# LFY1998/IPDM-PyTorch

Measured on AMD Instinct MI355X. Metric: CT slices/s (full proj+img partial-diffusion sample), higher is better.
Workload: dtype f32

## Files before the change

### ipdm-pytorch_amd/csrc/attn_bx3.hip

```cpp
#include "unet_kernels.h"
#include "attn_common.h"

using namespace ipdm;
using namespace ipdm::attn;

typedef float f32x16 __attribute__((ext_vector_type(16)));
typedef unsigned u32x4 __attribute__((ext_vector_type(4)));
typedef __bf16 bf16x8 __attribute__((ext_vector_type(8)));
typedef __bf16 bf16x2 __attribute__((ext_vector_type(2)));

namespace {

constexpr int D = 64;
constexpr int KT = 32;
constexpr int KP = 72;
constexpr int VP = 40;
constexpr int KPLANE = KT * KP, VPLANE = D * VP;
constexpr int STAGE = 3 * KPLANE + 3 * VPLANE;
constexpr int PCHUNK = 256;
constexpr int TILE_CHUNKS = 6 * PCHUNK;

__device__ inline unsigned pk_bf16(float a, float b)
{
    return __builtin_bit_cast(unsigned, bf16x2{(__bf16)a, (__bf16)b});
}
struct Split3 { unsigned h[3]; };
__device__ inline Split3 split3(float a, float b)
{
    Split3 s;
    s.h[0] = pk_bf16(a, b);
    const float ra = a - __builtin_bit_cast(float, s.h[0] << 16), rb = b - __builtin_bit_cast(float, s.h[0] & 0xffff0000u);
    s.h[1] = pk_bf16(ra, rb);
    const float qa = ra - __builtin_bit_cast(float, s.h[1] << 16), qb = rb - __builtin_bit_cast(float, s.h[1] & 0xffff0000u);
    s.h[2] = pk_bf16(qa, qb);
    return s;
}

__device__ inline f32x16 mma(u32x4 a, u32x4 b, f32x16 c)
{
    return __builtin_amdgcn_mfma_f32_32x32x16_bf16(__builtin_bit_cast(bf16x8, a), __builtin_bit_cast(bf16x8, b), c, 0, 0, 0);
}
template <bool FIRST>
__device__ inline f32x16 mma6(const u32x4 (&a)[3], const u32x4 (&b)[3], f32x16 c)
{
    if (FIRST) {
        const f32x16 zero = {0, 0, 0, 0, 0, 0, 0, 0, 0, 0, 0, 0, 0, 0, 0, 0};
        c = mma(a[0], b[2], zero);
        asm volatile("" ::"v"(a[0]), "v"(b[2]));
    } else {
        c = mma(a[0], b[2], c);
    }
    c = mma(a[2], b[0], c);
    c = mma(a[1], b[1], c);
    c = mma(a[0], b[1], c);
    c = mma(a[1], b[0], c);
    return mma(a[0], b[0], c);
}

__global__ void __launch_bounds__(256) attention_presplit_kernel(const float *__restrict__ qkv, u32x4 *__restrict__ planes, int heads, int T)
{
    constexpr int FP = KT + 1;
    __shared__ float kf[D * FP], vf[D * FP];
    const int bh = blockIdx.y, b = bh / heads, head = bh % heads;
    const float *qp = qkv + ((size_t)b * heads * 3 * D + (size_t)head * 3 * D) * T;
    const int s0 = blockIdx.x * KT, tid = threadIdx.x;
    {
        const int key = tid & 31, c0 = tid >> 5;
        const bool in = s0 + key < T;
#pragma unroll
        for (int r = 0; r < 8; ++r) {
            const int c = c0 + 8 * r;
            kf[c * FP + key] = in ? qp[(size_t)(D + c) * T + s0 + key] : 0.0f;
            vf[c * FP + key] = in ? qp[(size_t)(2 * D + c) * T + s0 + key] : 0.0f;
        }
    }
    __syncthreads();
    u32x4 *pt = planes + ((size_t)bh * gridDim.x + blockIdx.x) * TILE_CHUNKS + tid;
    const int ks = tid >> 3, kg = tid & 7, vc = tid >> 2, vg = tid & 3;
    const int vkey = 16 * (vg >> 1) + 4 * (vg & 1);
    u32x4 hk[3], hv[3];
#pragma unroll
    for (int e = 0; e < 8; e += 2) {
        const Split3 sk = split3(kf[(8 * kg + e) * FP + ks], kf[(8 * kg + e + 1) * FP + ks]);
        const Split3 sv = split3(vf[vc * FP + vkey + 8 * (e >> 2) + (e & 3)], vf[vc * FP + vkey + 8 * (e >> 2) + (e & 3) + 1]);
#pragma unroll
        for (int p = 0; p < 3; ++p) { hk[p][e / 2] = sk.h[p]; hv[p][e / 2] = sv.h[p]; }
    }
#pragma unroll
    for (int p = 0; p < 3; ++p) {
        pt[p * PCHUNK] = hk[p];
        pt[(3 + p) * PCHUNK] = hv[p];
    }
}

template <bool ZSEQ, bool PRE>
__global__ void __launch_bounds__(384, 3) attention_bx3_kernel(const float *__restrict__ qkv, float *__restrict__ out, int heads, int T,
                                                                float scale, int zsplit, float *__restrict__ part, int zseq,
                                                                const u32x4 *__restrict__ planes)
{
    __shared__ __attribute__((aligned(16))) unsigned short lds[2 * STAGE];
    const int bh = blockIdx.y;
    const int b = bh / heads, head = bh % heads;
    const float *qp = qkv + ((size_t)b * heads * 3 * D + (size_t)head * 3 * D) * T;
    const int ntiles = (T + KT - 1) / KT;
    const int nslice = ZSEQ ? zseq : zsplit;
    const int tps = 2 * (((T + 63) / 64 + nslice - 1) / nslice);
    const int it0 = ZSEQ ? 0 : blockIdx.z * tps, it1 = ZSEQ ? ntiles : min(ntiles, it0 + tps);

    if (__builtin_amdgcn_readfirstlane(threadIdx.x >> 6) >= 4) {
        if constexpr (PRE) {
            const int tid = threadIdx.x - 256;
            const __amdgpu_buffer_rsrc_t rs = __builtin_amdgcn_make_buffer_rsrc((void *)(planes + (size_t)bh * ntiles * TILE_CHUNKS), 0,
                                                                                  ntiles * TILE_CHUNKS * 16, 0x00020000);
            int ko[2], vo[2];
#pragma unroll
            for (int n = 0; n < 2; ++n) {
                const int j = tid + 128 * n;
                ko[n] = (j >> 3) * KP + 8 * (j & 7);
                vo[n] = 3 * KPLANE + (j >> 2) * VP + 8 * (j & 3);
            }
            u32x4 r[12];
            const auto load = [&](int it) {
#pragma unroll
                for (int i = 0; i < 12; ++i)
                    r[i] = __builtin_bit_cast(u32x4, __builtin_amdgcn_raw_buffer_load_b128(rs, tid * 16, (it * TILE_CHUNKS + 128 * i) * 16, 0));
            };
            const auto store = [&](int it) {
                unsigned short *st = lds + (it & 1) * STAGE;
#pragma unroll
                for (int i = 0; i < 6; ++i) {
                    *reinterpret_cast<u32x4 *>(st + (i >> 1) * KPLANE + ko[i & 1]) = r[i];
                    *reinterpret_cast<u32x4 *>(st + (i >> 1) * VPLANE + vo[i & 1]) = r[6 + i];
                }
            };
            if (it0 < it1) load(it0);
            for (int it = it0; it < it1; ++it) {
                store(it);
                if (it + 1 < it1) load(it + 1);
                __syncthreads();
            }
            return;
        }
        const int tid = threadIdx.x - 256;
        const __amdgpu_buffer_rsrc_t rs = __builtin_amdgcn_make_buffer_rsrc((void *)qp, 0, 3 * D * T * 4, 0x00020000);
        int ks[2], kg[2], koff[2], vg[2], vc[2], vkey[2], voff[2];
#pragma unroll
        for (int n = 0; n < 2; ++n) {
            const int idx = tid + 128 * n;
            ks[n] = idx & 31;
            kg[n] = idx >> 5;
            koff[n] = (8 * kg[n] * T + ks[n]) * 4;
            vg[n] = idx & 3;
            vc[n] = idx >> 2;
            vkey[n] = 16 * (vg[n] >> 1) + 4 * (vg[n] & 1);
            voff[n] = (vc[n] * T + vkey[n]) * 4;
        }
        float kr[2][8], vr[2][8];
        const auto load = [&](int it) {
            const int s0 = it * KT;
            if (s0 + KT <= T) {
#pragma unroll
                for (int n = 0; n < 2; ++n)
#pragma unroll
                    for (int e = 0; e < 8; ++e) {
                        kr[n][e] = __builtin_bit_cast(float, __builtin_amdgcn_raw_buffer_load_b32(rs, koff[n], (D * T + s0 + e * T) * 4, 0));
                        vr[n][e] = __builtin_bit_cast(float, __builtin_amdgcn_raw_buffer_load_b32(rs, voff[n], (2 * D * T + s0 + 8 * (e >> 2) + (e & 3)) * 4, 0));
                    }
            } else {
#pragma unroll
                for (int n = 0; n < 2; ++n)
#pragma unroll
                    for (int e = 0; e < 8; ++e) {
                        const int ko = s0 + ks[n] >= T ? 0x7fffffff : koff[n];
                        const int vo = s0 + vkey[n] + 8 * (e >> 2) + (e & 3) >= T ? 0x7fffffff : voff[n];
                        kr[n][e] = __builtin_bit_cast(float, __builtin_amdgcn_raw_buffer_load_b32(rs, ko, (D * T + s0 + e * T) * 4, 0));
                        vr[n][e] = __builtin_bit_cast(float, __builtin_amdgcn_raw_buffer_load_b32(rs, vo, (2 * D * T + s0 + 8 * (e >> 2) + (e & 3)) * 4, 0));
                    }
            }
        };
        const auto store = [&](int it) {
            unsigned short *st = lds + (it & 1) * STAGE;
#pragma unroll
            for (int n = 0; n < 2; ++n) {
                u32x4 hk[3], hv[3];
#pragma unroll
                for (int e = 0; e < 8; e += 2) {
                    const Split3 sk = split3(kr[n][e], kr[n][e + 1]), sv = split3(vr[n][e], vr[n][e + 1]);
#pragma unroll
                    for (int p = 0; p < 3; ++p) { hk[p][e / 2] = sk.h[p]; hv[p][e / 2] = sv.h[p]; }
                }
#pragma unroll
                for (int p = 0; p < 3; ++p) {
                    *reinterpret_cast<u32x4 *>(st + p * KPLANE + ks[n] * KP + 8 * kg[n]) = hk[p];
                    *reinterpret_cast<u32x4 *>(st + 3 * KPLANE + p * VPLANE + vc[n] * VP + 8 * vg[n]) = hv[p];
                }
            }
        };
        if (it0 < it1) load(it0);
        for (int it = it0; it < it1; ++it) {
            store(it);
            if (it + 1 < it1) load(it + 1);
            __syncthreads();
        }
        return;
    }

    const int tid = threadIdx.x, lane = tid & 63, wave = tid >> 6;
    const int l31 = lane & 31, lh = lane >> 5;
    const int t = blockIdx.x * 128 + wave * 32 + l31;
    u32x4 q[4][3];
#pragma unroll
    for (int kb = 0; kb < 4; ++kb) {
        float x[8];
#pragma unroll
        for (int e = 0; e < 8; ++e) x[e] = t < T ? qp[(size_t)(16 * kb + 8 * lh + e) * T + t] * (scale * scale) : 0.0f;
#pragma unroll
        for (int e = 0; e < 8; e += 2) {
            const Split3 s = split3(x[e], x[e + 1]);
#pragma unroll
            for (int p = 0; p < 3; ++p) q[kb][p][e / 2] = s.h[p];
        }
    }
    f32x16 o[2];
#pragma unroll
    for (int cb = 0; cb < 2; ++cb)
#pragma unroll
        for (int r = 0; r < 16; ++r) o[cb][r] = 0.0f;
    float m_run = -INFINITY, l_run = 0.0f;
    f32x16 num[ZSEQ ? 2 : 1];
    float M_all = -INFINITY, den = 0.0f;
#pragma unroll
    for (int cb = 0; cb < (ZSEQ ? 2 : 1); ++cb)
#pragma unroll
        for (int r = 0; r < 16; ++r) num[cb][r] = 0.0f;
    int slice_end = it0 + tps;
    u32x4 v[2][3] = {}, pp[2][3] = {};
    const auto reserve = [&]() {
        asm volatile("" ::"v"(v[0][0]), "v"(v[0][1]), "v"(v[0][2]), "v"(v[1][0]), "v"(v[1][1]), "v"(v[1][2]), "v"(pp[1][0]), "v"(pp[1][1]), "v"(pp[1][2]));
    };

    for (int it = it0; it < it1; ++it) {
        const int s0 = it * KT;
        __syncthreads();
        reserve();
        const unsigned short *st = lds + (it & 1) * STAGE;
        f32x16 sacc;
        u32x4 k[3];
        {
            const unsigned short *krow = st + l31 * KP + 8 * lh;
#pragma unroll
            for (int kb = 0; kb < 4; ++kb) {
#pragma unroll
                for (int p = 0; p < 3; ++p) k[p] = *reinterpret_cast<const u32x4 *>(krow + p * KPLANE + 16 * kb);
                sacc = kb == 0 ? mma6<true>(k, q[kb], sacc) : mma6<false>(k, q[kb], sacc);
            }
        }
        __builtin_amdgcn_sched_barrier(0);
        if (s0 + KT > T) {
#pragma unroll
            for (int r = 0; r < 16; ++r)
                if (s0 + crow(r, lh) >= T) sacc[r] = -INFINITY;
        }
        float mx = sacc[0];
#pragma unroll
        for (int r = 1; r < 16; ++r) mx = fmaxf(mx, sacc[r]);
        mx = halves_max(mx);
        const float m_new = fmaxf(m_run, mx);
        const float alpha = __builtin_amdgcn_exp2f((m_run - m_new) * LOG2E);
        float rs0 = 0.0f, rs1 = 0.0f;
#pragma unroll
        for (int r = 0; r < 16; r += 2) {
            sacc[r] = __builtin_amdgcn_exp2f((sacc[r] - m_new) * LOG2E);
            sacc[r + 1] = __builtin_amdgcn_exp2f((sacc[r + 1] - m_new) * LOG2E);
            rs0 += sacc[r];
            rs1 += sacc[r + 1];
        }
        const float rs = halves_sum(rs0 + rs1);
        asm volatile("" ::"v"(k[0]), "v"(k[1]), "v"(k[2]));
        l_run = l_run * alpha + rs;
        m_run = m_new;
        if (__any(alpha != 1.0f)) {
#pragma unroll
            for (int cb = 0; cb < 2; ++cb)
#pragma unroll
                for (int r = 0; r < 16; ++r) o[cb][r] *= alpha;
        }
#pragma unroll
        for (int kb = 0; kb < 2; ++kb)
#pragma unroll
            for (int e = 0; e < 8; e += 2) {
                const Split3 s = split3(sacc[8 * kb + e], sacc[8 * kb + e + 1]);
#pragma unroll
                for (int p = 0; p < 3; ++p) pp[kb][p][e / 2] = s.h[p];
            }
        __builtin_amdgcn_sched_barrier(0);
#pragma unroll
        for (int cb = 0; cb < 2; ++cb) {
            const unsigned short *vrow = st + 3 * KPLANE + (cb * 32 + l31) * VP + 8 * lh;
#pragma unroll
            for (int kb = 0; kb < 2; ++kb)
#pragma unroll
                for (int p = 0; p < 3; ++p) v[kb][p] = *reinterpret_cast<const u32x4 *>(vrow + p * VPLANE + 16 * kb);
#pragma unroll
            for (int kb = 0; kb < 2; ++kb) o[cb] = mma6<false>(v[kb], pp[kb], o[cb]);
        }
        __builtin_amdgcn_sched_barrier(0);
        if constexpr (ZSEQ) if (it + 1 == slice_end || it + 1 == it1) {
            const SliceWeights w = slice_weights(M_all, m_run);
            den = slice_fold(den, l_run, w);
#pragma unroll
            for (int cb = 0; cb < 2; ++cb)
#pragma unroll
                for (int r = 0; r < 16; ++r) { num[cb][r] = slice_fold(num[cb][r], o[cb][r], w); o[cb][r] = 0.0f; }
            m_run = -INFINITY;
            l_run = 0.0f;
            slice_end += tps;
        }
    }
    if (t >= T) { reserve(); return; }
    if (zsplit > 1) {
        float *pq = part + ((size_t)blockIdx.z * gridDim.y + bh) * (D + 2) * T;
#pragma unroll
        for (int cb = 0; cb < 2; ++cb)
#pragma unroll
            for (int r = 0; r < 16; ++r) pq[(size_t)(cb * 32 + crow(r, lh)) * T + t] = o[cb][r];
        if (lh == 0) { pq[(size_t)D * T + t] = m_run; pq[(size_t)(D + 1) * T + t] = l_run; }
        reserve();
        return;
    }
    float *op = out + ((size_t)b * heads * D + (size_t)head * D) * T;
    const float inv = 1.0f / (ZSEQ ? den : l_run);
#pragma unroll
    for (int cb = 0; cb < 2; ++cb)
#pragma unroll
        for (int r = 0; r < 16; ++r) op[(size_t)(cb * 32 + crow(r, lh)) * T + t] = (ZSEQ ? num[ZSEQ ? cb : 0][r] : o[cb][r]) * inv;
    reserve();
}

}

namespace ipdm {

size_t attention_planes_floats(int B, int heads, int d, int T)
{
    if (d != D || opt(OPT_ATTN_EXACT_F32) || opt(OPT_ATTN_LEGACY) || opt(OPT_ATTN_NO_PRESPLIT)) return 0;
    return (size_t)B * heads * cdiv(T, KT) * TILE_CHUNKS * 4;
}

void attention_bx3_launch(const float *qkv, float *out, int B, int heads, int T, float scale, int Z, bool seq, float *scratch,
                          float *planes, hipStream_t st)
{
    const dim3 grid(cdiv(T, 128), B * heads, seq ? 1 : Z);
    u32x4 *pl = reinterpret_cast<u32x4 *>(planes);
    if (pl) hipLaunchKernelGGL(attention_presplit_kernel, dim3(cdiv(T, KT), B * heads), dim3(256), 0, st, qkv, pl, heads, T);
    if (seq) {
        if (pl) hipLaunchKernelGGL((attention_bx3_kernel<true, true>), grid, dim3(384), 0, st, qkv, out, heads, T, scale, 1, (float *)nullptr, Z, pl);
        else hipLaunchKernelGGL((attention_bx3_kernel<true, false>), grid, dim3(384), 0, st, qkv, out, heads, T, scale, 1, (float *)nullptr, Z, pl);
    } else {
        if (pl) hipLaunchKernelGGL((attention_bx3_kernel<false, true>), grid, dim3(384), 0, st, qkv, out, heads, T, scale, Z, scratch, 1, pl);
        else hipLaunchKernelGGL((attention_bx3_kernel<false, false>), grid, dim3(384), 0, st, qkv, out, heads, T, scale, Z, scratch, 1, pl);
    }
}

}
```

### ipdm-pytorch_amd/csrc/common.h

```cpp
#pragma once
#include <hip/hip_runtime.h>
#include <cstdarg>
#include <cstdio>
#include <cstring>
#include <string>
#include <vector>
#include "../../include/ipdm_hip.h"

namespace ipdm {

void set_error(const char *fmt, ...);

#define IPDM_HIP_CHECK(expr)                                                                   \
    do {                                                                                       \
        hipError_t e_ = (expr);                                                                \
        if (e_ != hipSuccess) {                                                                \
            ipdm::set_error("%s failed: %s (%s:%d)", #expr, hipGetErrorString(e_), __FILE__,  \
                            __LINE__);                                                         \
            return IPDM_ERR_HIP;                                                               \
        }                                                                                      \
    } while (0)

#define IPDM_REQUIRE(cond, ...)                   \
    do {                                          \
        if (!(cond)) {                            \
            ipdm::set_error(__VA_ARGS__);         \
            return IPDM_ERR_INVALID;              \
        }                                         \
    } while (0)

#define IPDM_LAUNCH_CHECK() IPDM_HIP_CHECK(hipGetLastError())

static inline int cdiv(long a, long b) { return (int)((a + b - 1) / b); }
static inline size_t align_up(size_t v, size_t a) { return (v + a - 1) / a * a; }

enum Opt {
    OPT_CONV_NO_UP2,
    OPT_CONV_NO_WUP2,
    OPT_CONV_LEGACY, OPT_CONV1X1_LEGACY, OPT_CONVS2_LEGACY,
    OPT_CONV_NO_DIRECT, OPT_DIRECT_NO_PLANAR, OPT_DIRECT_MAX_CIN, OPT_DIRECT_NO_S2, OPT_DIRECT_NO_SKIP_FUSE,
    OPT_CONV_DBG, OPT_CONV_VEC4_STRICT, OPT_CONV_NO_SPLITK, OPT_CONV_NO_WINO, OPT_WINO_V1, OPT_WINO2_MIN_TILES, OPT_CONV1X1_NO_QUARTER, OPT_CONV_NO_PW, OPT_PW_ITEM, OPT_PW_FORCE,
    OPT_CONV_NM,
    OPT_GN_TWO_STAGE, OPT_GN_UNFUSED,
    OPT_UNET_TRANSPOSE,
    OPT_ATTN_NO_KVSPLIT, OPT_ATTN_LEGACY, OPT_ATTN_NO_ZSEQ,
    OPT_ART_PER_VIEW,
    OPT_CONV_BF16X3,
    OPT_ATTN_EXACT_F32,
    OPT_ATTN_NO_PRESPLIT,
    OPT_COUNT
};
int opt(Opt o);
bool opt_per_call(int o);
const char *opt_name(int o);
void opt_snapshot(int (&dst)[OPT_COUNT]);
int opt_changed_since(const int (&rec)[OPT_COUNT]);
std::vector<int> opt_per_call_values();

int ensure_dynamic_lds(const void *kernel, size_t bytes);
int device_cu_count();

int unet_io_channels(const ipdm_unet *net, int *cin, int *cout);

__device__ inline double wave_sum(double v)
{
#pragma unroll
    for (int o = 32; o > 0; o >>= 1) v += __shfl_down(v, o, 64);
    return v;
}
__device__ inline float wave_sum(float v)
{
#pragma unroll
    for (int o = 32; o > 0; o >>= 1) v += __shfl_down(v, o, 64);
    return v;
}
__device__ inline float wave_max(float v)
{
#pragma unroll
    for (int o = 32; o > 0; o >>= 1) v = fmaxf(v, __shfl_down(v, o, 64));
    return v;
}

}
```

### ipdm-pytorch_amd/csrc/common.hip

```cpp
#include <cctype>
#include <cstdlib>
#include <mutex>
#include <strings.h>
#include <set>
#include <utility>
#include "common.h"

namespace ipdm {
static thread_local char g_err[512] = "";
void set_error(const char *fmt, ...)
{
    va_list ap;
    va_start(ap, fmt);
    vsnprintf(g_err, sizeof(g_err), fmt, ap);
    va_end(ap);
}

namespace {
std::mutex g_attr_mu;
std::set<std::pair<const void *, int>> g_attr_done;
int g_cus[64];
}

namespace {
struct OptDef { const char *name; int def; bool per_call; int lo = 0, hi = 1; };
const OptDef g_opt_def[OPT_COUNT] = {
    {"conv_no_up2", 0, true},
    {"conv_no_wup2", 0, true},
    {"conv_legacy", 0, false}, {"conv1x1_legacy", 0, false}, {"convs2_legacy", 0, false},
    {"conv_no_direct", 0, false}, {"direct_no_planar", 0, false},
    {"direct_max_cin", 160, false, 0, 160},
    {"direct_no_s2", 0, false}, {"direct_no_skip_fuse", 0, true},
    {"conv_dbg", 0, true, 0, 0x3ff}, {"conv_vec4_strict", 0, false}, {"conv_no_splitk", 0, false},
    {"conv_no_wino", 0, true}, {"wino_v1", 0, true}, {"wino2_min_tiles", 192, true, 0, 1 << 24},
    {"conv1x1_no_quarter", 0, true}, {"conv_no_pw", 0, true}, {"pw_item", 0, true, 0, 2}, {"pw_force", 0, true}, {"conv_nm", 0, true, 0, 2},
    {"gn_two_stage", 0, true}, {"gn_unfused", 0, true},
    {"unet_transpose", -1, true, -1, 1},
    {"attn_no_kvsplit", 0, false}, {"attn_legacy", 0, false}, {"attn_no_zseq", 0, true},
    {"art_per_view", 0, true},
    {"conv_bf16x3", 0, true},
    {"attn_exact_f32", 0, true},
    {"attn_no_presplit", 0, true},
};
bool opt_value_ok(int i, int v)
{
    return v >= g_opt_def[i].lo && v <= g_opt_def[i].hi;
}
std::mutex g_opt_mu;
int g_opt_val[OPT_COUNT];
bool g_opt_init = false;

void opt_init_locked()
{
    if (g_opt_init) return;
    for (int i = 0; i < OPT_COUNT; ++i) {
        char env[64] = "IPDM_";
        size_t n = 5;
        for (const char *c = g_opt_def[i].name; *c && n + 1 < sizeof(env); ++c) env[n++] = (char)toupper((unsigned char)*c);
        env[n] = 0;
        const char *e = getenv(env);
        g_opt_val[i] = g_opt_def[i].def;
        if (e) {
            char *end = nullptr;
            const long v = strtol(e, &end, 10);
            const int want = (end != e) ? (int)v : 1;
            if (opt_value_ok(i, want)) g_opt_val[i] = want;
            else fprintf(stderr, "libipdm_hip: %s=%s is outside the option's range [%d, %d]: ignored\n", env, e, g_opt_def[i].lo, g_opt_def[i].hi);
        }
    }
    g_opt_init = true;
}
}

int opt(Opt o)
{
    std::lock_guard<std::mutex> lk(g_opt_mu);
    opt_init_locked();
    return g_opt_val[o];
}
bool opt_per_call(int o) { return g_opt_def[o].per_call; }
const char *opt_name(int o) { return g_opt_def[o].name; }
void opt_snapshot(int (&dst)[OPT_COUNT])
{
    std::lock_guard<std::mutex> lk(g_opt_mu);
    opt_init_locked();
    for (int i = 0; i < OPT_COUNT; ++i) dst[i] = g_opt_val[i];
}
std::vector<int> opt_per_call_values()
{
    std::lock_guard<std::mutex> lk(g_opt_mu);
    opt_init_locked();
    std::vector<int> v;
    for (int i = 0; i < OPT_COUNT; ++i)
        if (g_opt_def[i].per_call) v.push_back(g_opt_val[i]);
    return v;
}
int opt_changed_since(const int (&rec)[OPT_COUNT])
{
    std::lock_guard<std::mutex> lk(g_opt_mu);
    opt_init_locked();
    for (int i = 0; i < OPT_COUNT; ++i)
        if (!g_opt_def[i].per_call && g_opt_val[i] != rec[i]) return i;
    return -1;
}
static int opt_find(const char *name)
{
    if (!name) return -1;
    if (!strncmp(name, "IPDM_", 5) || !strncmp(name, "ipdm_", 5)) name += 5;
    for (int i = 0; i < OPT_COUNT; ++i)
        if (!strcasecmp(name, g_opt_def[i].name)) return i;
    return -1;
}

int ensure_dynamic_lds(const void *kernel, size_t bytes)
{
    int dev = 0;
    IPDM_HIP_CHECK(hipGetDevice(&dev));
    std::lock_guard<std::mutex> lk(g_attr_mu);
    if (g_attr_done.count({kernel, dev})) return IPDM_OK;
    IPDM_HIP_CHECK(hipFuncSetAttribute(kernel, hipFuncAttributeMaxDynamicSharedMemorySize, (int)bytes));
    g_attr_done.insert({kernel, dev});
    return IPDM_OK;
}

int device_cu_count()
{
    int dev = 0, v = 0;
    if (hipGetDevice(&dev) != hipSuccess || dev < 0 || dev >= 64) return 256;
    std::lock_guard<std::mutex> lk(g_attr_mu);
    if (!g_cus[dev])
        g_cus[dev] = (hipDeviceGetAttribute(&v, hipDeviceAttributeMultiprocessorCount, dev) == hipSuccess && v > 0) ? v : 256;
    return g_cus[dev];
}
}

extern "C" const char *ipdm_last_error(void) { return ipdm::g_err; }
extern "C" int ipdm_abi_version(void) { return IPDM_ABI_VERSION; }

extern "C" int ipdm_set_option(const char *name, int value)
{
    const int i = ipdm::opt_find(name);
    IPDM_REQUIRE(i >= 0, "ipdm_set_option: unknown option '%s'", name ? name : "(null)");
    IPDM_REQUIRE(ipdm::opt_value_ok(i, value), "ipdm_set_option: %s = %d is outside [%d, %d]", ipdm::g_opt_def[i].name, value,
                 ipdm::g_opt_def[i].lo, ipdm::g_opt_def[i].hi);
    std::lock_guard<std::mutex> lk(ipdm::g_opt_mu);
    ipdm::opt_init_locked();
    ipdm::g_opt_val[i] = value;
    return IPDM_OK;
}

extern "C" int ipdm_get_option(const char *name, int *value)
{
    const int i = ipdm::opt_find(name);
    IPDM_REQUIRE(i >= 0 && value, "ipdm_get_option: unknown option '%s'", name ? name : "(null)");
    *value = ipdm::opt((ipdm::Opt)i);
    return IPDM_OK;
}
```

Before: 2.161.

## Software-pipeline attention loop: overlap next tile's QK^T with current softmax and PV

Adds a pipelined variant of the bf16x3 attention kernel for the presplit, non-sequential path. The producer warps now stage K and V halves of each tile one barrier apart. The compute warps interleave the next tile's QK^T MMAs with the current tile's exp/split and PV MMAs, using sched_barrier pinning and register-reservation asm. The goal is to hide softmax and LDS latency behind matrix work. The cost is more register pressure and complex scheduling, and an env option can disable it.

After: 2.187 (median of 6 runs). 1.2% higher.

```diff
diff --git a/ipdm-pytorch_amd/csrc/attn_bx3.hip b/ipdm-pytorch_amd/csrc/attn_bx3.hip
--- a/ipdm-pytorch_amd/csrc/attn_bx3.hip
+++ b/ipdm-pytorch_amd/csrc/attn_bx3.hip
@@ -1,5 +1,7 @@
 #include "unet_kernels.h"
 #include "attn_common.h"
+#include "attn_pipe_schedule.h"
+#include <type_traits>
 
 using namespace ipdm;
 using namespace ipdm::attn;
@@ -57,6 +59,15 @@
     return mma(a[0], b[0], c);
 }
 
+template <int FROM, int TO, class F>
+__device__ inline void static_for(F &&f)
+{
+    if constexpr (FROM < TO) {
+        f(std::integral_constant<int, FROM>{});
+        static_for<FROM + 1, TO>(f);
+    }
+}
+
 __global__ void __launch_bounds__(256) attention_presplit_kernel(const float *__restrict__ qkv, u32x4 *__restrict__ planes, int heads, int T)
 {
     constexpr int FP = KT + 1;
@@ -93,11 +104,13 @@
     }
 }
 
-template <bool ZSEQ, bool PRE>
+template <bool ZSEQ, bool PRE, bool PIPE>
 __global__ void __launch_bounds__(384, 3) attention_bx3_kernel(const float *__restrict__ qkv, float *__restrict__ out, int heads, int T,
                                                                 float scale, int zsplit, float *__restrict__ part, int zseq,
                                                                 const u32x4 *__restrict__ planes)
 {
+    static_assert(PRE || !PIPE, "the pipelined loop copies planes");
+    static_assert(!ZSEQ || !PIPE, "the pipelined loop does not fit the slice walk's registers");
     __shared__ __attribute__((aligned(16))) unsigned short lds[2 * STAGE];
     const int bh = blockIdx.y;
     const int b = bh / heads, head = bh % heads;
@@ -106,6 +119,7 @@
     const int nslice = ZSEQ ? zseq : zsplit;
     const int tps = 2 * (((T + 63) / 64 + nslice - 1) / nslice);
     const int it0 = ZSEQ ? 0 : blockIdx.z * tps, it1 = ZSEQ ? ntiles : min(ntiles, it0 + tps);
+    const int npipe = max(it1 - it0, 0);
 
     if (__builtin_amdgcn_readfirstlane(threadIdx.x >> 6) >= 4) {
         if constexpr (PRE) {
@@ -133,6 +147,34 @@
                     *reinterpret_cast<u32x4 *>(st + (i >> 1) * VPLANE + vo[i & 1]) = r[6 + i];
                 }
             };
+            if constexpr (PIPE) {
+                const auto load_half = [&](int it, int h) {
+#pragma unroll
+                    for (int i = 6 * h; i < 6 * h + 6; ++i)
+                        r[i] = __builtin_bit_cast(u32x4, __builtin_amdgcn_raw_buffer_load_b128(rs, tid * 16, (it * TILE_CHUNKS + 128 * i) * 16, 0));
+                };
+                const auto store_k = [&](int it) {
+                    unsigned short *st = lds + attn_pipe::slot(it) * STAGE;
+#pragma unroll
+                    for (int i = 0; i < 6; ++i) *reinterpret_cast<u32x4 *>(st + (i >> 1) * KPLANE + ko[i & 1]) = r[i];
+                };
+                const auto store_v = [&](int it) {
+                    unsigned short *st = lds + attn_pipe::slot(it) * STAGE;
+#pragma unroll
+                    for (int i = 0; i < 6; ++i) *reinterpret_cast<u32x4 *>(st + (i >> 1) * VPLANE + vo[i & 1]) = r[6 + i];
+                };
+                if (npipe > 0) load_half(attn_pipe::k_stored(it0, npipe, 0), 0);
+                for (int b = 0; b < attn_pipe::barriers(npipe); ++b) {
+                    const int ks = attn_pipe::k_stored(it0, npipe, b), vs = attn_pipe::v_stored(it0, npipe, b);
+                    if (ks != attn_pipe::NONE) store_k(ks);
+                    if (vs != attn_pipe::NONE) store_v(vs);
+                    const int kl = attn_pipe::k_loaded(it0, npipe, b), vl = attn_pipe::v_loaded(it0, npipe, b);
+                    if (kl != attn_pipe::NONE) load_half(kl, 0);
+                    if (vl != attn_pipe::NONE) load_half(vl, 1);
+                    __syncthreads();
+                }
+                return;
+            }
             if (it0 < it1) load(it0);
             for (int it = it0; it < it1; ++it) {
                 store(it);
@@ -239,6 +281,135 @@
         asm volatile("" ::"v"(v[0][0]), "v"(v[0][1]), "v"(v[0][2]), "v"(v[1][0]), "v"(v[1][1]), "v"(v[1][2]), "v"(pp[1][0]), "v"(pp[1][1]), "v"(pp[1][2]));
     };
 
+    if constexpr (PIPE) {
+        f32x16 sacc = {};
+        float mx_c = 0.0f, m_new_c = 0.0f, alpha_c = 1.0f;
+        const auto row_max_alpha = [&]() {
+            mx_c = sacc[0];
+#pragma unroll
+            for (int r = 1; r < 16; ++r) mx_c = fmaxf(mx_c, sacc[r]);
+            mx_c = halves_max(mx_c);
+            m_new_c = fmaxf(m_run, mx_c);
+            alpha_c = __builtin_amdgcn_exp2f((m_run - m_new_c) * LOG2E);
+        };
+        u32x4 ka[2] = {}, pb[2] = {};
+        const auto interval = [&](auto has_s, auto has_pv, int b) {
+            constexpr bool HAS_S = decltype(has_s)::value, HAS_PV = decltype(has_pv)::value;
+            constexpr bool PIN = HAS_PV;
+            const int it = attn_pipe::v_read(it0, npipe, b), s0 = it * KT;
+            f32x16 snext;
+            u32x4 k[3], k0n;
+            if constexpr (HAS_PV) asm volatile("" ::"v"(ka[0]), "v"(ka[1]), "v"(pb[0]), "v"(pb[1]));
+            const unsigned short *krow = lds + (HAS_S ? attn_pipe::slot(attn_pipe::k_read(it0, npipe, b)) : 0) * STAGE + l31 * KP + 8 * lh;
+            const auto kterm = [&](int p, int kb) { return *reinterpret_cast<const u32x4 *>(krow + p * KPLANE + 16 * kb); };
+            float rs0 = 0.0f, rs1 = 0.0f;
+            float ra[4], rb[4];
+            unsigned h0[4];
+            const auto split_a = [&](int kb, int i) {
+                const float x = sacc[8 * kb + 2 * i], y = sacc[8 * kb + 2 * i + 1];
+                h0[i] = pk_bf16(x, y);
+                ra[i] = x - __builtin_bit_cast(float, h0[i] << 16);
+                rb[i] = y - __builtin_bit_cast(float, h0[i] & 0xffff0000u);
+            };
+            const auto split_b = [&](int kb, int i) {
+                const unsigned h1 = pk_bf16(ra[i], rb[i]);
+                const float qa = ra[i] - __builtin_bit_cast(float, h1 << 16), qb = rb[i] - __builtin_bit_cast(float, h1 & 0xffff0000u);
+                pp[kb][0][i] = h0[i];
+                pp[kb][1][i] = h1;
+                pp[kb][2][i] = pk_bf16(qa, qb);
+            };
+            if constexpr (HAS_PV && !HAS_S) if (s0 + KT > T) {
+#pragma unroll
+                for (int r = 0; r < 16; ++r)
+                    if (s0 + crow(r, lh) >= T) sacc[r] = -INFINITY;
+                row_max_alpha();
+            }
+            const float m_new = m_new_c, alpha = alpha_c;
+            if constexpr (HAS_PV) {
+                if (__any(alpha != 1.0f)) {
+#pragma unroll
+                    for (int cb = 0; cb < 2; ++cb)
+#pragma unroll
+                        for (int r = 0; r < 16; ++r) o[cb][r] *= alpha;
+                }
+                __builtin_amdgcn_sched_barrier(0);
+            }
+            if constexpr (HAS_S) {
+#pragma unroll
+                for (int p = 0; p < 3; ++p) k[p] = kterm(p, 0);
+            }
+            static_for<0, 24>([&](auto gc) {
+                constexpr int g = decltype(gc)::value, kb = g / 6, j = g % 6;
+                if constexpr (HAS_S) {
+                    constexpr int TA[6] = {0, 2, 1, 0, 1, 0}, TB[6] = {2, 0, 1, 1, 0, 0};
+                    if constexpr (g == 0) {
+                        const f32x16 zero = {0, 0, 0, 0, 0, 0, 0, 0, 0, 0, 0, 0, 0, 0, 0, 0};
+                        snext = mma(k[0], q[0][2], zero);
+                        asm volatile("" ::"v"(k[0]), "v"(q[0][2]));
+                    } else {
+                        snext = mma(k[TA[j]], q[kb][TB[j]], snext);
+                    }
+                    if constexpr (g >= 2) asm volatile("" ::"v"(ka[g % 2]));
+                    ka[g % 2] = k[TA[j]];
+                    if constexpr (kb < 3 && j == 1) { k[2] = kterm(2, kb + 1); k0n = kterm(0, kb + 1); }
+                    if constexpr (kb < 3 && j == 4) k[1] = kterm(1, kb + 1);
+                    if constexpr (kb < 3 && j == 5) k[0] = k0n;
+                }
+                if constexpr (HAS_PV) {
+                    if constexpr (g < 16) {
+                        sacc[g] = __builtin_amdgcn_exp2f((sacc[g] - m_new) * LOG2E);
+                        if constexpr (g % 2 == 0) rs0 += sacc[g]; else rs1 += sacc[g];
+                    } else if constexpr (g == 16) {
+                        const float rs = halves_sum(rs0 + rs1);
+                        l_run = l_run * alpha + rs;
+                        m_run = m_new;
+                    }
+                    if constexpr (g >= 2 && g < 10 && g % 2 == 0) split_a(0, (g - 2) / 2);
+                    if constexpr (g >= 3 && g < 11 && g % 2 == 1) split_b(0, (g - 3) / 2);
+                }
+                if constexpr (PIN) __builtin_amdgcn_sched_barrier(0);
+            });
+            if constexpr (HAS_PV) {
+                const unsigned short *vt = lds + attn_pipe::slot(it) * STAGE + 3 * KPLANE + l31 * VP + 8 * lh;
+                const auto vterms = [&](int cb, int kb) {
+#pragma unroll
+                    for (int p = 0; p < 3; ++p) v[cb][p] = *reinterpret_cast<const u32x4 *>(vt + cb * 32 * VP + p * VPLANE + 16 * kb);
+                };
+                vterms(0, 0);
+
+                static_for<0, 24>([&](auto gc) {
+                    constexpr int g = decltype(gc)::value, kb = g / 12, cb = (g / 6) % 2, j = g % 6;
+                    constexpr int TA[6] = {0, 2, 1, 0, 1, 0}, TB[6] = {2, 0, 1, 1, 0, 0};
+                    o[cb] = mma(v[cb][TA[j]], pp[kb][TB[j]], o[cb]);
+                    if constexpr (HAS_S || g >= 2) asm volatile("" ::"v"(ka[g % 2]));
+                    if constexpr (g >= 2) asm volatile("" ::"v"(pb[g % 2]));
+                    ka[g % 2] = v[cb][TA[j]];
+                    pb[g % 2] = pp[kb][TB[j]];
+                    if constexpr (g == 2) vterms(1, 0);
+                    if constexpr (kb == 0 && j == 5) vterms(cb, 1);
+                    if constexpr (g < 8 && g % 2 == 0) split_a(1, g / 2);
+                    if constexpr (g < 8 && g % 2 == 1) split_b(1, g / 2);
+                    if constexpr (HAS_S && g == 12) { sacc = snext; row_max_alpha(); }
+                    if constexpr (PIN) __builtin_amdgcn_sched_barrier(0);
+                });
+                __builtin_amdgcn_sched_barrier(0);
+            }
+            if constexpr (HAS_S && !HAS_PV) {
+                sacc = snext;
+                row_max_alpha();
+            }
+        };
+        if (attn_pipe::barriers(npipe) > 0) {
+            __syncthreads();
+            interval(std::true_type{}, std::false_type{}, 0);
+            for (int b = 1; b <= attn_pipe::steady(npipe); ++b) {
+                __syncthreads();
+                interval(std::true_type{}, std::true_type{}, b);
+            }
+            __syncthreads();
+            interval(std::false_type{}, std::true_type{}, attn_pipe::barriers(npipe) - 1);
+        }
+    } else
     for (int it = it0; it < it1; ++it) {
         const int s0 = it * KT;
         __syncthreads();
@@ -353,13 +524,18 @@
     const dim3 grid(cdiv(T, 128), B * heads, seq ? 1 : Z);
     u32x4 *pl = reinterpret_cast<u32x4 *>(planes);
     if (pl) hipLaunchKernelGGL(attention_presplit_kernel, dim3(cdiv(T, KT), B * heads), dim3(256), 0, st, qkv, pl, heads, T);
+    const bool pipe = pl && !seq && !opt(OPT_ATTN_NO_PIPELINE);
+    const auto launch = [&](auto kernel, int zsplit, float *part, int zseq) {
+        hipLaunchKernelGGL(kernel, grid, dim3(384), 0, st, qkv, out, heads, T, scale, zsplit, part, zseq, pl);
+    };
     if (seq) {
-        if (pl) hipLaunchKernelGGL((attention_bx3_kernel<true, true>), grid, dim3(384), 0, st, qkv, out, heads, T, scale, 1, (float *)nullptr, Z, pl);
-        else hipLaunchKernelGGL((attention_bx3_kernel<true, false>), grid, dim3(384), 0, st, qkv, out, heads, T, scale, 1, (float *)nullptr, Z, pl);
+        if (pl) launch(attention_bx3_kernel<true, true, false>, 1, nullptr, Z);
+        else launch(attention_bx3_kernel<true, false, false>, 1, nullptr, Z);
     } else {
-        if (pl) hipLaunchKernelGGL((attention_bx3_kernel<false, true>), grid, dim3(384), 0, st, qkv, out, heads, T, scale, Z, scratch, 1, pl);
-        else hipLaunchKernelGGL((attention_bx3_kernel<false, false>), grid, dim3(384), 0, st, qkv, out, heads, T, scale, Z, scratch, 1, pl);
-    }
-}
-
-}
+        if (pipe) launch(attention_bx3_kernel<false, true, true>, Z, scratch, 1);
+        else if (pl) launch(attention_bx3_kernel<false, true, false>, Z, scratch, 1);
+        else launch(attention_bx3_kernel<false, false, false>, Z, scratch, 1);
+    }
+}
+
+}
diff --git a/ipdm-pytorch_amd/csrc/attn_pipe_schedule.h b/ipdm-pytorch_amd/csrc/attn_pipe_schedule.h
--- /dev/null
+++ b/ipdm-pytorch_amd/csrc/attn_pipe_schedule.h
@@ -0,0 +1,22 @@
+#pragma once
+
+namespace ipdm {
+namespace attn_pipe {
+
+constexpr int NONE = -1;
+
+constexpr int barriers(int n) { return n > 0 ? n + 1 : 0; }
+constexpr int steady(int n) { return n > 0 ? n - 1 : 0; }
+
+constexpr int k_stored(int it0, int n, int b) { return b >= 0 && b < n ? it0 + b : NONE; }
+constexpr int v_stored(int it0, int n, int b) { return b >= 1 && b <= n ? it0 + b - 1 : NONE; }
+constexpr int k_loaded(int it0, int n, int b) { return k_stored(it0, n, b + 1); }
+constexpr int v_loaded(int it0, int n, int b) { return v_stored(it0, n, b + 1); }
+
+constexpr int k_read(int it0, int n, int b) { return b >= 0 && b < n ? it0 + b : NONE; }
+constexpr int v_read(int it0, int n, int b) { return b >= 1 && b <= n ? it0 + b - 1 : NONE; }
+
+constexpr int slot(int tile) { return tile & 1; }
+
+}
+}
diff --git a/ipdm-pytorch_amd/csrc/common.h b/ipdm-pytorch_amd/csrc/common.h
--- a/ipdm-pytorch_amd/csrc/common.h
+++ b/ipdm-pytorch_amd/csrc/common.h
@@ -48,6 +48,7 @@
     OPT_CONV_BF16X3,
     OPT_ATTN_EXACT_F32,
     OPT_ATTN_NO_PRESPLIT,
+    OPT_ATTN_NO_PIPELINE,
     OPT_COUNT
 };
 int opt(Opt o);
diff --git a/ipdm-pytorch_amd/csrc/common.hip b/ipdm-pytorch_amd/csrc/common.hip
--- a/ipdm-pytorch_amd/csrc/common.hip
+++ b/ipdm-pytorch_amd/csrc/common.hip
@@ -41,6 +41,7 @@
     {"conv_bf16x3", 0, true},
     {"attn_exact_f32", 0, true},
     {"attn_no_presplit", 0, true},
+    {"attn_no_pipeline", 0, true},
 };
 bool opt_value_ok(int i, int v)
 {
```
